# hupe1980/vecgo

Measured on AMD Instinct MI355X. Metric: QPS at recall@10≥0.95, 1M×768 HNSW+PQ; PQ-ADC HBM GB/s vs peak, higher is better.
Workload: dtype f32; 1 GPU; flat_exact_l2_1Mx768_top10 (BASELINE configs[1]): MFMA GEMM nomination + exact re-score + proof; operating_point=flat_exact, rows=1000000, dim=768, k=10, parallelism=1 GPU

## Files before the change

vecgo_amd/csrc/k_flat.hip:

```cpp
#include <algorithm>

#include "vg_device.hpp"
#include "vg_exact.hpp"
#include "vg_cand_replay.hpp"
#include "vg_flat_gemm.hpp"
#include "vg_internal.hpp"
#include "vg_nominate.hpp"
#include "vg_search.hpp"

namespace vg {

struct GemmOperands {
    const float *a, *b;
    int64_t n;
    int dim_words;
    const float *norms;
    bool bf16, dma;
};
struct NomCall {
    hipStream_t st;
    bool dot;
    GemmOperands ops;
    int64_t cnt;
    const uint8_t *mask;
// ... 4 lines not shown
    const NomCall &c;
    const float *queries;
    float *scores = nullptr;
    int tile_stride = 1;
    int64_t out_cols = 0;
    const float *thr = nullptr;
    int thr_stride = 0, thr_off = 0;
    int *counts = nullptr;
    uint64_t *cand = nullptr;
    int cap = 0;
    int cus = 256;
    int *counts_wide = nullptr;
    int skip_stride = 0;
    bool split = false;
    bool screen = false;
    const uint32_t *tile_active = nullptr;

    explicit GemmArgs(const NomCall &call) : c(call), queries(call.ops.a) {}
    static GemmArgs sample(const NomCall &c, float *sc, int stride, int64_t cols)
    {
        GemmArgs a(c);
        a.scores = sc, a.tile_stride = stride, a.out_cols = cols;
        return a;
    }
    static GemmArgs append(const NomCall &c, const float *thr, int sel_k, int *counts, uint64_t *cand, int cap)
    {
        GemmArgs a(c);
        a.thr = thr, a.thr_stride = sel_k, a.thr_off = sel_k - 1, a.counts = counts, a.cand = cand, a.cap = cap;
        return a;
    }
    GemmArgs &wide(int *lines, int compute_units) { return counts_wide = lines, cus = compute_units, *this; }
    GemmArgs &skipping(int stride) { return skip_stride = stride, *this; }
    GemmArgs &split_tile(const uint32_t *image) { return queries = reinterpret_cast<const float *>(image), split = true, *this; }
    GemmArgs &screen_tile() { return screen = true, *this; }
    GemmArgs &retry(const uint32_t *active) { return tile_active = active, *this; }
};
constexpr int kCountLine = 32;
static bool gemm_runs_split(bool fused, bool bf16, bool dma, int64_t nq, int dim, int cap, int thr_stride)
{
    return fused && !bf16 && dma && nq > kGemmBM && dim % kGemmBK == 0 && nq * static_cast<int64_t>(cap) < (int64_t(1) << 31) &&
           thr_stride < 65536 && !hook(kHookFlatNoSplit);
}
static float split_gemm_eps(bool dot, int dim)
{
    const float m = static_cast<float>(3 * dim + 16) * 5.9604645e-8f;
    return dot ? 1.5001f * 1.52587890625e-5f + 2.52f * m : 3.0002f * 1.52587890625e-5f + 4.03f * m;
}
static float screen_gemm_eps(bool dot, int dim)
{
    const float m = static_cast<float>(dim + 16) * 5.9604645e-8f;
    return dot ? 0.00390625f + 7.62939453125e-6f + 2.52f * m : 0.0078125f + 1.52587890625e-5f + 4.03f * m;
}
float bf16_filter_eps(bool dot) { return (dot ? 0.00390625f : 0.0078125f) * 1.02f; }
static bool gemm_skips_sample(bool dma, int64_t nq, bool bf16, bool split = false)
{
    if (bf16 || split || hook(kHookFlatRescoreSample)) return false;
    return !(dma && nq <= 3 * kG32BM && !hook(kHookFlatNoSmallTile));
}
__global__ void counts_narrow_kernel(const int *__restrict__ wide, int64_t nq, int *__restrict__ counts)
{
    const int64_t q = static_cast<int64_t>(blockIdx.x) * blockDim.x + threadIdx.x;
    if (q < nq) counts[q] = wide[q * kCountLine];
}

template <class Kern, class... Args>
static int32_t launch_lds(Kern kern, dim3 grid, dim3 threads, size_t lds, hipStream_t st, Args... args)
{
// ... 17 lines not shown
    const NomCall &c = a.c;
    const bool dma = c.ops.dma, bf16 = c.ops.bf16;
    const hipStream_t st = c.st;
    const int skip = MODE == 2 ? a.skip_stride : 0;
    VG_CHECK(skip == 0 || (skip > 1 && gemm_skips_sample(dma, c.cnt, bf16, a.split)), VG_ERR_INVALID_ARG, "launch_gemm: skip_stride on a kernel without it");
    const int64_t mt = (c.cnt + kGemmBM - 1) / kGemmBM, nt = (c.ops.n + kGemmBN - 1) / kGemmBN;
    const int64_t tiles = skip ? nt - gemm_skip_sampled_tiles(nt, skip) : (nt + a.tile_stride - 1) / a.tile_stride;
    const dim3 grid(static_cast<unsigned>(mt * ((tiles + 7) / 8) * 8)), threads(kGemmThreads);
    auto big_grid = [&](int64_t bnt ) {
        const int64_t bmt = (c.cnt + kBigBM - 1) / kBigBM;
        const int64_t slots = bmt * ((bnt + 7) / 8) * 8, per_cu = std::max(a.cus / 8, 1) * 8;
        return dim3(static_cast<unsigned>(std::min(slots, per_cu)));
    };
    auto launch_big = [&](auto kern, size_t lds, auto... extra) -> int32_t {
        if (a.counts_wide && !a.tile_active) VG_HIP(hipMemsetAsync(a.counts_wide, 0, sizeof(int) * static_cast<size_t>(c.cnt) * kCountLine, st));
        VG_TRY(launch_lds(kern, big_grid((c.ops.n + kBigBN - 1) / kBigBN), dim3(kBigThreads), lds, st, a.queries, c.cnt, c.ops.b, c.ops.n,
                          c.ops.dim_words, c.ops.norms, a.thr, a.thr_stride, a.thr_off, a.counts_wide ? a.counts_wide : a.counts, a.cand, a.cap, c.mask,
                          c.mask_stride, a.counts_wide ? kCountLine : 1, extra...));
        if (a.counts_wide)
            VG_LAUNCH(counts_narrow_kernel, dim3(static_cast<unsigned>((c.cnt + 255) / 256)), dim3(256), 0, st, a.counts_wide, c.cnt, a.counts);
        return VG_OK;
    };
    auto launch_tile = [&](auto kern, dim3 blocks, size_t lds, auto... last) -> int32_t {
        return launch_lds(kern, blocks, threads, lds, st, a.queries, c.cnt, c.ops.b, c.ops.n, c.ops.dim_words, c.ops.norms, a.scores, a.tile_stride, a.out_cols, a.thr,
                          a.thr_stride, a.thr_off, a.counts, a.cand, a.cap, c.mask, c.mask_stride, last...);
    };
    auto launch_128 = [&](auto kern, size_t lds, int last) { return launch_tile(kern, grid, lds, last); };
    auto launch_g32 = [&](auto kern, size_t lds) { return launch_tile(kern, dim3(static_cast<unsigned>(tiles)), lds); };
    constexpr int M = MODE == 0 ? 1 : MODE;
    const int rb = static_cast<int>((c.cnt + kG32BM - 1) / kG32BM);
    if constexpr (MODE == 1) {
        if (a.split) {
            VG_CHECK(!bf16 && gemm_runs_split(true, false, dma, c.cnt, c.ops.dim_words, 0, 0), VG_ERR_INVALID_ARG, "launch_gemm: sample tile on a call without it");
            return launch_lds(flat_gemm_sample_big_kernel<DOT, 3>, big_grid((tiles + 1) / 2), dim3(kBigThreads), big_lds_bytes<3>(), st, a.queries, c.cnt,
                              c.ops.b, c.ops.n, c.ops.dim_words, c.ops.norms, a.scores, a.tile_stride, a.out_cols, c.mask, c.mask_stride);
        }
    }
    if (MODE == 2 && a.split) {
        VG_CHECK(!bf16 && gemm_runs_split(true, false, dma, c.cnt, c.ops.dim_words, a.cap, a.thr_stride), VG_ERR_INVALID_ARG, "launch_gemm: split tile on a call without it");
        if (a.screen) return launch_big(flat_gemm_screen_big_kernel<DOT, 3>, big_lds_bytes<3>());
        VG_CHECK(!a.tile_active || (c.cnt <= 32 * kBigBM && a.counts_wide), VG_ERR_INVALID_ARG, "launch_gemm: tile_active is one word, with wide counters");
        note_flat_split_launch();
        return launch_big(flat_gemm_split_big_kernel<DOT, 3>, big_lds_bytes<3>(), a.tile_active);
    }
    if (skip && tiles == 0) return VG_OK;
    if (bf16) {
        if (c.cnt <= 4 * kG32BM && !hook(kHookFlatNoSmallTile)) return with_g32_tile<DOT, M, true>(rb, launch_g32);
        if (MODE == 2 && c.cnt > kGemmBM && c.cnt * static_cast<int64_t>(a.cap) < (int64_t(1) << 31) && a.thr_stride < 65536 &&
            !hook(kHookFlatNoBigTile)) {
            const bool two = hook(kHookFlatBigTile2);
            auto kern = two ? flat_gemm_bf16_big_kernel<DOT, 2> : hook(kHookFlatBigEarlyB) ? flat_gemm_bf16_big_kernel<DOT, 3, 512> : flat_gemm_bf16_big_kernel<DOT, 3>;
            return launch_big(kern, two ? big_lds_bytes<2>() : big_lds_bytes<3>());
        }
        return launch_128(flat_gemm_dma_kernel<DOT, M, 0, true>, kDmaLdsBytes, 0);
    }
    if (dma && MODE != 0 && c.cnt <= 3 * kG32BM && !hook(kHookFlatNoSmallTile)) return with_g32_tile<DOT, M, false>(rb, launch_g32);
    if (dma) return launch_128(flat_gemm_dma_kernel<DOT, MODE>, kDmaLdsBytes, skip);
    return launch_128(flat_gemm_kernel<DOT, MODE>, kGemmLdsBytes, skip);
}

template <int MODE>
static int32_t launch_gemm(const GemmArgs &a)
{
    return a.c.dot ? launch_gemm_t<true, MODE>(a) : launch_gemm_t<false, MODE>(a);
}

__global__ void f32_to_bf16_pad_kernel(const float *__restrict__ src, int64_t rows, int dim, int dim_pad, uint16_t *__restrict__ dst)
{
    const int64_t i = static_cast<int64_t>(blockIdx.x) * blockDim.x + threadIdx.x;
    if (i >= rows * dim_pad) return;
    const int64_t r = i / dim_pad;
    const int j = static_cast<int>(i - r * dim_pad);
    const uint32_t u = j < dim ? __float_as_uint(src[r * dim + j]) : 0u;
    uint16_t v;
    if ((u & 0x7F800000u) == 0x7F800000u && (u & 0x007FFFFFu) != 0)
        v = static_cast<uint16_t>((u >> 16) | 0x0040u);
    else
        v = static_cast<uint16_t>((u + 0x7FFFu + ((u >> 16) & 1u)) >> 16);
    dst[i] = v;
}

__global__ void flat_split_queries_kernel(const float *__restrict__ src, int64_t rows, int dim, uint32_t *__restrict__ dst)
{
    const int64_t i = static_cast<int64_t>(blockIdx.x) * blockDim.x + threadIdx.x;
    const int half = dim / 2;
    if (i >= rows * half) return;
    const int64_t r = i / half;
    const int p = static_cast<int>(i - r * half), s = p >> 4, w = p & 15;
    const float2 v = *reinterpret_cast<const float2 *>(src + r * dim + 32 * s + 2 * w);
    uint32_t hi, lo;
    split2_bf16(v.x, v.y, hi, lo);
    dst[r * dim + 32 * s + w] = hi;
    dst[r * dim + 32 * s + 16 + w] = lo;
}

__global__ __launch_bounds__(256) void flat_todo_kernel(const int *__restrict__ flags, const int *__restrict__ always,
                                                        int cnt, int *__restrict__ todo,
                                                        unsigned long long *__restrict__ stats, const int *__restrict__ counts)
{
    __shared__ int part[256];
    __shared__ unsigned long long appended[256];
    const int tid = threadIdx.x;
    const int per = (cnt + 255) / 256;
    const int lo = tid * per < cnt ? tid * per : cnt, hi = lo + per < cnt ? lo + per : cnt;
    if (!flags) {
        if (tid == 0) atomicAdd(&stats[0], static_cast<unsigned long long>(cnt));
        return;
    }
    const bool all = *always != 0;
    int mine = 0;
    unsigned long long app = 0;
    for (int i = lo; i < hi; i++) {
        mine += (all || flags[i] != 0);
        if (counts) app += static_cast<unsigned long long>(counts[i]);
    }
    part[tid] = mine;
    appended[tid] = app;
    __syncthreads();
    if (tid == 0) {
        int run = 0;
        app = 0;
        for (int t = 0; t < 256; t++) {
            const int c = part[t];
            part[t] = run;
            run += c;
            app += appended[t];
// ... 545 lines not shown
    {
        cols = cols_;
        slices = slices_ ? slices_ : select_slices(cols, 4096, 64);
        nom.sel_k = sel_k;
        nom.cap = cap;
        c.take(sc, sampled ? cnt * cols : 1);
        c.take(partial, cnt * slices * sel_k);
        c.take(sid, cnt * sel_k);
        c.take(nom.thr, cnt * sel_k);
        c.take(nom.counts, cnt);
        c.take(nom.cand, cnt * cap);
        c.take(nom.cand_id, cnt * kFlatKc);
        c.take(nom.cand_sc, cnt * kFlatKc);
    }
};
static int32_t launch_flat_select(const NomScratch &s, int64_t cnt, int sel_k, hipStream_t st)
{
    VG_LAUNCH(flat_select_kernel, dim3(s.slices, static_cast<unsigned>(cnt)), dim3(kSelThreads), 0, st, s.sc, s.cols, s.slices, sel_k, s.partial);
    return VG_OK;
}
static int32_t select_thresholds(const NomScratch &s, int64_t cnt, int sel_k, uint32_t *ids, float *thr, hipStream_t st)
{
    VG_TRY(launch_flat_select(s, cnt, sel_k, st));
    return launch_topk_merge(s.partial, cnt, s.slices, sel_k, false, ids, thr, st);
}
static int32_t sample_thresholds(const NomCall &c, const NomScratch &s, int stride, int sel_k, float *thr, bool sampled, const uint32_t *image = nullptr,
                                 int cus = 0)
{
    if (!sampled) {
        VG_LAUNCH(fill_f32_kernel, dim3(static_cast<unsigned>((c.cnt * sel_k + 255) / 256)), dim3(256), 0, c.st, thr, c.cnt * sel_k, INFINITY);
        return VG_OK;
    }
    GemmArgs a = GemmArgs::sample(c, s.sc, stride, s.cols);
    if (image) a.split_tile(image).wide(nullptr, cus);
    VG_TRY(launch_gemm<1>(a));
    return select_thresholds(s, c.cnt, sel_k, s.sid, thr, c.st);
}
static int32_t launch_flat_pick(const ProbeNominated &nom, int64_t cnt, const int *only, hipStream_t st)
{
    VG_LAUNCH(flat_pick_kernel, dim3(static_cast<unsigned>(cnt)), dim3(256), 0, st, nom.cand, nom.counts, nom.cap, kFlatKc, nom.cand_id, nom.cand_sc, only);
    return VG_OK;
}
static int32_t launch_flat_verify(bool dot, int k, const vg_index *idx, const float *queries, int64_t cnt, const ProbeNominated &nom,
                                  float eps_extra, uint32_t *ids, float *scores, int *fail, const int *only, hipStream_t st)
{
    return with_metric(dot, [&](auto dot_c) -> int32_t {
        constexpr bool DOT = decltype(dot_c)::value;
        const dim3 grid(static_cast<unsigned>(cnt)), threads(256);
        if (nom.thr && k > 64)
            VG_LAUNCH(flat_verify_sort_kernel<DOT>, grid, threads, sizeof(uint64_t) * static_cast<size_t>(nom.cap), st, idx->d_vectors, idx->dim, queries,
                      idx->d_norm_max, nom.cand, nom.counts, nom.cap, k, ids, scores, fail, nom.thr, nom.sel_k, nom.sel_k - 1, eps_extra);
        else if (nom.thr && k > kGemmMaxK)
            VG_LAUNCH(flat_verify_all_kernel<DOT>, grid, threads, 0, st, idx->d_vectors, idx->dim, queries, idx->d_norm_max, nom.cand, nom.counts,
                      nom.cap, k, ids, scores, fail, nom.thr, nom.sel_k, nom.sel_k - 1, eps_extra);
        else
            VG_LAUNCH(flat_verify_kernel<DOT>, grid, threads, 0, st, idx->d_vectors, idx->n, idx->dim, queries, idx->d_norm_max, nom.cand_id,
                      nom.cand_sc, kFlatKc, k, ids, scores, fail, nom.thr, nom.sel_k, nom.sel_k - 1, nom.counts, nom.cap, eps_extra, only);
        return VG_OK;
    });
}

struct FlatCall {
    vg_index *idx;
    int k;
    hipStream_t st;
    bool dot;
    const float *q;
    int64_t nq;
    const uint8_t *mask;
    int64_t mask_stride;
    uint32_t *oid;
    float *osc;
    int64_t n = idx->n;
    int dim = idx->dim;
    FlatCall range(int64_t q0, int64_t cnt) const
    {
        FlatCall r = *this;
        r.q += q0 * dim, r.nq = cnt, r.oid += q0 * k, r.osc += q0 * k;
        if (mask) r.mask += q0 * mask_stride;
        return r;
    }
    NomCall nom() const { return {st, dot, fp32_operands(idx, q, !hook(kHookFlatNoDma)), nq, mask, mask_stride}; }
};
constexpr int kFlatCap = 4096;
constexpr int kFlatSampleStride = 64;
static int exact_slices(int64_t n) { return static_cast<int>(std::min<int64_t>(256, std::max<int64_t>(1, n / 64))); }
struct FlatScratch : NomScratch {
    bool fused;
    bool use_sample;
    bool bf16;
    bool may_split;
    int ex_slices, pk;
    int64_t qc;
    int *flags, *todo;
    uint64_t *fpartial, *min_keys;
    uint32_t *fid;
    float *fsc;
    uint16_t *qbf;
    int *counts_wide;
    uint32_t *tile_active;
    FlatScratch(const FlatCall &c, bool unfused, char *base) : fused(!unfused), use_sample(fused && c.n > kFlatCap)
    {
        bf16 = c.idx->d_vectors_bf16 != nullptr && fused && !hook(kHookFlatNoDma);
        const int sel_k = !fused ? kFlatKc : c.k <= 64 ? 8 : std::min(64, std::max(8, (3 * c.k + 63) / 64));
        ex_slices = exact_slices(c.n);
        pk = std::min(c.k, 64);
        qc = fused ? 4096 : (int64_t(2) << 30) / (c.n * 4);
        if (qc > 4096) qc = 4096;
        if (qc >= kGemmBM) qc = (qc / kGemmBM) * kGemmBM;
        if (qc < 1) qc = 1;
        if (qc > c.nq) qc = c.nq;
        may_split = gemm_runs_split(fused, bf16, true, qc, c.dim, kFlatCap, sel_k);
        Carve cv{base};
        carve(cv, qc, fused ? sample_cols(c.n, kFlatSampleStride) : c.n, sel_k, fused ? kFlatCap : 0, !fused || use_sample);
        cv.take(flags, qc + 1);
        cv.take(todo, qc + 1);
        cv.take(fpartial, qc * ex_slices * pk);
        cv.take(fid, qc * pk);
        cv.take(fsc, qc * pk);
        cv.take(min_keys, qc);
        cv.take(qbf, bf16 ? qc * c.idx->vectors_bf16_dim : may_split ? 2 * qc * c.dim : 0);
        cv.take(counts_wide, bf16 || may_split ? qc * kCountLine : 0);
        cv.take(tile_active, may_split ? 1 : 0);
        bytes = cv.off;
    }
};

static int32_t flat_scan_small(const FlatCall &c)
{
    const int slices = static_cast<int>(std::min<int64_t>(4 * c.idx->ctx->compute_units, std::max<int64_t>(1, c.n / 64)));
    ArenaCall ar(c.idx->ctx, c.st);
    const int i_partial = ar.add(sizeof(uint64_t) * static_cast<size_t>(c.nq) * slices * c.k);
    VG_TRY(ar.commit());
    uint64_t *partial = ar.get<uint64_t>(i_partial);
    const size_t lds = sizeof(float) * static_cast<size_t>(kScanQB) * c.dim + 4 * 64 * sizeof(uint64_t) + 64;
    for (int64_t q0 = 0; q0 < c.nq; q0 += kScanQB) {
        const int cnt = static_cast<int>(std::min<int64_t>(kScanQB, c.nq - q0));
        ProfScope prof(c.idx->ctx, "flat_scan", c.st);
        auto kern = c.dot ? flat_scan_mq_kernel<true> : flat_scan_mq_kernel<false>;
        VG_LAUNCH(kern, dim3(slices), dim3(256), lds, c.st, c.idx->d_vectors, c.n, c.dim, c.q + q0 * c.dim, cnt, slices, c.k, partial + q0 * slices * c.k);
    }
    VG_TRY(launch_topk_merge(partial, c.nq, slices, c.k, c.dot, c.oid, c.osc, c.st));
    return launch_flat_todo(nullptr, nullptr, static_cast<int>(c.nq), nullptr, c.idx->d_flat_stats, c.st);
}

static int32_t launch_flat_exact(const FlatCall &c, const int *todo, int ex_slices, int kk, uint64_t *fpartial, const uint64_t *floor_keys)
{
    const unsigned slots = static_cast<unsigned>(std::min<int64_t>(c.nq, kExactSlots));
    auto kern = c.dot ? flat_exact_kernel<true> : flat_exact_kernel<false>;
    VG_LAUNCH(kern, dim3(ex_slices, slots), dim3(256), 0, c.st, c.idx->d_vectors, c.n, c.dim, c.q, todo, ex_slices, kk, fpartial, floor_keys, c.mask,
              c.mask_stride);
    return VG_OK;
}
static int32_t flat_exact_every_query(const FlatCall &call)
// ... 30 lines not shown
        VG_TRY(launch_flat_select(s, c.nq, kFlatKc, c.st));
    }
    VG_TRY(launch_topk_merge(s.partial, c.nq, s.slices, kFlatKc, false, s.nom.cand_id, s.nom.cand_sc, c.st));
    ProbeNominated nom = s.nom;
    nom.thr = nullptr;
    return launch_flat_verify(c.dot, c.k, c.idx, c.q, c.nq, nom, 0.0f, c.oid, c.osc, s.flags, nullptr, c.st);
}

static int32_t flat_screen_retry(const FlatCall &c, const NomCall &nc, const FlatScratch &s)
{
    const ProbeNominated &nom = s.nom;
    VG_LAUNCH(flat_retry_prepare_kernel, dim3(1), dim3(kBigBM), 0, c.st, s.flags, hook(kHookFlatScreenFail), static_cast<int>(c.nq), nom.thr,
              nom.sel_k, nom.sel_k - 1, nom.counts, s.counts_wide, s.tile_active, c.idx->d_flat_stats);
    {
        ProfScope prof(c.idx->ctx, "flat_retry", c.st);
        VG_TRY(launch_gemm<2>(GemmArgs::append(nc, nom.thr, nom.sel_k, nom.counts, nom.cand, nom.cap)
                                  .wide(s.counts_wide, c.idx->ctx->compute_units)
                                  .split_tile(reinterpret_cast<const uint32_t *>(s.qbf))
                                  .retry(s.tile_active)));
    }
    VG_TRY(launch_flat_pick(nom, c.nq, s.flags, c.st));
    return launch_flat_verify(c.dot, c.k, c.idx, c.q, c.nq, nom, split_gemm_eps(c.dot, c.dim), c.oid, c.osc, s.flags, s.flags, c.st);
}

static int32_t flat_fused_chunk(const FlatCall &c, const FlatScratch &s)
{
    const vg_index *idx = c.idx;
    const ProbeNominated &nom = s.nom;
    NomCall nc = c.nom();
    const bool split = gemm_runs_split(true, s.bf16, nc.ops.dma, c.nq, c.dim, nom.cap, nom.sel_k);
    const bool screen = gemm_runs_screen(split, c.k);
    const float eps_extra = screen ? screen_gemm_eps(c.dot, c.dim) : split ? split_gemm_eps(c.dot, c.dim) : s.bf16 ? bf16_filter_eps(c.dot) : 0.0f;
    if (s.bf16) VG_TRY(gemm_operands(c.q, c.nq, c.dim, c.n, idx->d_norms, idx->d_vectors_bf16, idx->vectors_bf16_dim, s.qbf, c.st, &nc.ops));
    const uint32_t *image = reinterpret_cast<const uint32_t *>(s.qbf);
    if (split)
        VG_LAUNCH(flat_split_queries_kernel, dim3(static_cast<unsigned>((c.nq * (c.dim / 2) + 255) / 256)), dim3(256), 0, c.st, c.q, c.nq, c.dim,
                  reinterpret_cast<uint32_t *>(s.qbf));
    VG_TRY(sample_thresholds(nc, s, kFlatSampleStride, nom.sel_k, nom.thr, s.use_sample, sample_runs_big(split, s.use_sample) ? image : nullptr,
                             idx->ctx->compute_units));
    if (s.bf16 || split) VG_LAUNCH(flat_thr_cap_kernel, dim3(nc.ucnt()), dim3(64), 0, c.st, nom.thr, nom.sel_k, c.q, c.dim, idx->d_norm_max);
    const bool once = s.use_sample && gemm_skips_sample(nc.ops.dma, c.nq, s.bf16, split);
    if (!once) VG_HIP(hipMemsetAsync(nom.counts, 0, sizeof(int) * static_cast<size_t>(c.nq), c.st));
    {
        ProfScope prof(idx->ctx, "flat_gemm", c.st);
        if (once)
            VG_LAUNCH(flat_sample_append_kernel, dim3(nc.ucnt()), dim3(kSampleAppendThreads), 0, c.st, s.sc, s.cols, kFlatSampleStride, nom.thr,
                      nom.sel_k, nom.sel_k - 1, nom.counts, nom.cand, nom.cap);
        GemmArgs a = GemmArgs::append(nc, nom.thr, nom.sel_k, nom.counts, nom.cand, nom.cap);
        a.wide(s.bf16 || split ? s.counts_wide : nullptr, idx->ctx->compute_units).skipping(once ? kFlatSampleStride : 0);
        if (split) a.split_tile(reinterpret_cast<const uint32_t *>(s.qbf));
        if (screen) a.screen_tile();
        VG_TRY(launch_gemm<2>(a));
    }
    if (c.k <= kGemmMaxK) VG_TRY(launch_flat_pick(nom, c.nq, nullptr, c.st));
    VG_TRY(launch_flat_verify(c.dot, c.k, idx, c.q, c.nq, nom, eps_extra, c.oid, c.osc, s.flags, nullptr, c.st));
    return screen ? flat_screen_retry(c, nc, s) : VG_OK;
}

static void flat_debug_counts(const FlatCall &c, int64_t q0, const FlatScratch &s)
{
    std::vector<int> hf(c.nq), hc(c.nq);
    (void)hipMemcpyAsync(hf.data(), s.flags, sizeof(int) * c.nq, hipMemcpyDeviceToHost, c.st);
    (void)hipMemcpyAsync(hc.data(), s.nom.counts, sizeof(int) * c.nq, hipMemcpyDeviceToHost, c.st);
    (void)hipStreamSynchronize(c.st);
    int64_t nf = 0, csum = 0, cmax = 0;
    for (int f : hf) nf += f != 0;
    for (int n : hc) { csum += n; cmax = std::max<int64_t>(cmax, n); }
    fprintf(stderr, "[vg_search_flat] chunk q0=%lld cnt=%lld: %lld queries failed the proof; "
            "appended candidates avg %.1f max %lld\n", (long long)q0, (long long)c.nq, (long long)nf,
            s.fused ? double(csum) / c.nq : 0.0, (long long)(s.fused ? cmax : 0));
}

static int32_t flat_fallback_pages(const FlatCall &c, const FlatScratch &s)
{
    const int *always = s.flags + s.qc;
    const dim3 grid(static_cast<unsigned>(c.nq));
    for (int off = 0; off < c.k; off += 64) {
        const int kk = std::min(64, c.k - off);
        VG_TRY(launch_flat_exact(c, s.todo, s.ex_slices, kk, s.fpartial, off ? s.min_keys : nullptr));
        VG_TRY(launch_topk_merge(s.fpartial, c.nq, s.ex_slices, kk, c.dot, s.fid, s.fsc, c.st, s.flags, always));
        if (c.k <= 64)
            VG_LAUNCH(flat_patch_kernel, grid, dim3(64), 0, c.st, s.flags, always, c.k, s.fid, s.fsc, c.oid, c.osc);
        else
            VG_LAUNCH(flat_page_patch_kernel, grid, dim3(64), 0, c.st, s.flags, always, c.k, off, kk, c.dot, s.fid, s.fsc, c.oid, c.osc, s.min_keys);
// ... 302 lines not shown
```

vecgo_amd/csrc/vg_flat_gemm.hpp:

```cpp
#pragma once

#include <hip/hip_runtime.h>

#include <cmath>
#include <cstdint>
#include <type_traits>

#include "vg_device.hpp"

namespace vg {

constexpr int kGemmBM = 128, kGemmBN = 128, kGemmBK = 32, kGemmLd = kGemmBK + 1;
constexpr int kGemmPasses = kGemmBM * kGemmBK / 4 / 256;
constexpr int kGemmThreads = 256;
constexpr int kGemmTile = kGemmBM * kGemmLd;
constexpr size_t kGemmLdsBytes = 4 * kGemmTile * sizeof(float);
using f32x16 = __attribute__((ext_vector_type(16))) float;

template <bool DOT, int MODE>
__device__ __forceinline__ void gemm_epilogue(const f32x16 (&acc)[2][2], float *lds_thr, float thr_reg,
                                              const float (&xn)[2], int tid, int lane, int wr, int wc, int64_t q0,
                                              int64_t nq, int64_t n0, int64_t n, int64_t tn,
                                              float *__restrict__ scores, int64_t out_cols,
                                              int *__restrict__ counts, uint64_t *__restrict__ cand, int cap,
// ... 438 lines not shown

struct GemmGroup {
    int64_t a_off, b_off;
    int32_t a_cnt, b_cnt;
};
template <bool DOT, int MODE, bool BF16 = false>
__global__ __launch_bounds__(kGemmThreads) void flat_gemm_dma_grouped_kernel(
    const GemmGroup *__restrict__ groups, const int64_t *__restrict__ first_block, int ngroups,
    const float *__restrict__ queries, const float *__restrict__ base, int dim, const float *__restrict__ norms,
    float *__restrict__ scores, int tile_stride, int64_t out_cols, const float *__restrict__ thr, int thr_stride, int thr_off,
    int *__restrict__ counts, uint64_t *__restrict__ cand, int cap, const uint8_t *__restrict__ mask , const int64_t *__restrict__ mask_off )
{
    const int64_t b = blockIdx.x;
    if (b >= first_block[ngroups]) return;
    int lo = 0, hi = ngroups - 1;
    while (lo < hi) {
        const int mid = (lo + hi + 1) >> 1;
        if (first_block[mid] <= b)
            lo = mid;
        else
            hi = mid - 1;
    }
    const GemmGroup g = groups[lo];
    if (g.a_cnt == 0 || g.b_cnt == 0) return;
    flat_gemm_dma_body<DOT, MODE, 0, BF16, true>(
        queries + g.a_off * dim, g.a_cnt, base + g.b_off * dim, g.b_cnt, dim, norms + g.b_off,
        scores ? scores + g.a_off * out_cols : nullptr, tile_stride, out_cols, thr ? thr + g.a_off * thr_stride : nullptr, thr_stride,
        thr_off, counts ? counts + g.a_off : nullptr, cand ? cand + g.a_off * cap : nullptr, cap, mask, 0, b - first_block[lo],
        static_cast<uint32_t>(g.b_off), mask ? mask_off + g.a_off : nullptr);
}

constexpr int kBigBM = 256, kBigBN = 256, kBigThreads = 512;
constexpr int kBigTile = kBigBM * kGemmBK;
template <int NB>
constexpr size_t big_lds_bytes() { return (2 + NB) * kBigTile * sizeof(float); }

__device__ __forceinline__ void big_split3(float x, uint32_t &p0, uint32_t &p1, uint32_t &p2)
{
    auto rne = [](float v) {
        const uint32_t u = __float_as_uint(v);
        return (u + 0x7FFFu + ((u >> 16) & 1u)) >> 16;
    };
    p0 = rne(x);
    const float r1 = x - __uint_as_float(p0 << 16);
    p1 = rne(r1);
    const float r2 = r1 - __uint_as_float(p1 << 16);
    p2 = rne(r2);
}
__device__ __forceinline__ int big_max3_i32(int a, int b, int c)
{
    int r;
    asm("v_max3_i32 %0, %1, %2, %3" : "=v"(r) : "v"(a), "v"(b), "v"(c));
    return r;
}

typedef __bf16 vg_bf16x2 __attribute__((ext_vector_type(2)));
typedef float vg_f32x2 __attribute__((ext_vector_type(2)));
__device__ __forceinline__ void split2_bf16(float a, float b, uint32_t &hi, uint32_t &lo)
{
    hi = __builtin_bit_cast(uint32_t, __builtin_convertvector(vg_f32x2{a, b}, vg_bf16x2));
    const float ra = a - __uint_as_float(hi << 16), rb = b - __uint_as_float(hi & 0xFFFF0000u);
    lo = __builtin_bit_cast(uint32_t, __builtin_convertvector(vg_f32x2{ra, rb}, vg_bf16x2));
}

enum { kBigImages = 0, kBigSplit = 1, kBigScreen = 2 };
template <bool DOT, int NB, int PROBE, int OPS, bool SAMPLE = false>
__device__ __forceinline__ void flat_gemm_big_body(
    const float *__restrict__ queries, int64_t nq, const float *__restrict__ base, int64_t n, int dim ,
    const float *__restrict__ norms, const float *__restrict__ thr, int thr_stride, int thr_off, int *__restrict__ counts,
    uint64_t *__restrict__ cand, int cap, const uint8_t *__restrict__ mask, int64_t mask_stride,
    int count_stride ,
    const uint32_t *__restrict__ tile_active = nullptr, float *__restrict__ scores = nullptr ,
    int tile_stride = 1, int64_t out_cols = 0)
{
    static_assert(NB == 2 || NB == 3, "two or three row-tile buffers");
    constexpr bool SPLIT = OPS != kBigImages;
    constexpr bool SCREEN = OPS == kBigScreen;
    extern __shared__ float gemm_lds[];
    const int mtiles = static_cast<int>((nq + kBigBM - 1) / kBigBM);
    const int ntiles = SAMPLE ? static_cast<int>((((n + kGemmBN - 1) / kGemmBN + tile_stride - 1) / tile_stride + 1) / 2)
                              : static_cast<int>((n + kBigBN - 1) / kBigBN);
    const int total = mtiles * ((ntiles + 7) / 8) * 8, G = static_cast<int>(gridDim.x), xcd = static_cast<int>(blockIdx.x & 7);
    const int dq = (G >> 3) / mtiles, dr = (G >> 3) % mtiles;
    struct Pos {
        int bt, quo, rem;
    };
    auto tm_of = [&](const Pos &p) { return p.rem; };
    auto tn_of = [&](const Pos &p) { return p.quo * 8 + xcd; };
    const uint32_t active = tile_active ? *tile_active : 0xFFFFFFFFu;
    auto hole = [&](const Pos &p) { return tn_of(p) >= ntiles || ((active >> (p.rem & 31)) & 1u) == 0; };
    auto step = [&](Pos &p) {
        do {
            p.bt += G;
            p.quo += dq;
            p.rem += dr;
            if (p.rem >= mtiles) {
                p.rem -= mtiles;
                p.quo++;
            }
        } while (p.bt < total && hole(p));
    };
    Pos pos0;
    pos0.bt = static_cast<int>(blockIdx.x);
    pos0.quo = (pos0.bt >> 3) / mtiles;
    pos0.rem = (pos0.bt >> 3) % mtiles;
    if (pos0.bt < total && hole(pos0)) step(pos0);
    if (pos0.bt >= total) return;
    int my_tiles = 0;
    for (Pos p = pos0; p.bt < total; step(p)) my_tiles++;

    const int tid = threadIdx.x;
    const int lane = tid & 63;
    const int wave = __builtin_amdgcn_readfirstlane(tid >> 6);
    const int wr = wave >> 2, wc = wave & 3;
    const int ksteps = dim / kGemmBK;
    const int S = my_tiles * ksteps;

    const int drow = wave * 8 + (lane >> 3);
    const int dgl = (lane & 7) ^ ((wave * 4 + (lane >> 4)) & 7);
    const uint32_t lds0 = static_cast<uint32_t>(reinterpret_cast<uintptr_t>(
        (__attribute__((address_space(3))) void *)gemm_lds));
    auto piece = [&](int buf, int p) {
        return static_cast<uint32_t>(__builtin_amdgcn_readfirstlane(
            static_cast<int>(lds0 + (buf * kBigTile + (p * 64 + wave * 8) * kGemmBK) * 4)));
    };
    Pos a_pos = pos0, b_pos = pos0;
    int a_k = 0, b_k = 0, ia = 0, ib = 0;
    const float *abase, *bbase, *bbase1 = nullptr;
    int a_last, b_last, b_last1 = 0;
    const uint32_t off0 = static_cast<uint32_t>((drow * dim + dgl * 4) * 4);
    auto set_a = [&](const Pos &ps) {
        const int64_t q0 = static_cast<int64_t>(tm_of(ps)) * kBigBM;
        abase = queries + q0 * dim;
        a_last = static_cast<int>(nq - q0 < kBigBM ? nq - q0 : kBigBM) - 1;
    };
    auto set_b = [&](const Pos &ps) {
        const int64_t n0 = static_cast<int64_t>(tn_of(ps)) * kBigBN;
        bbase = base + n0 * dim;
        b_last = static_cast<int>(n - n0 < kBigBN ? n - n0 : kBigBN) - 1;
    };
    auto half_row0 = [&](const Pos &ps, int hf) { return (static_cast<int64_t>(tn_of(ps)) * 2 + hf) * tile_stride * kGemmBN; };
    auto set_b_halves = [&](const Pos &ps) {
        const int64_t r0 = half_row0(ps, 0), r1 = half_row0(ps, 1);
        bbase = base + r0 * dim;
        b_last = static_cast<int>(n - r0 < kGemmBN ? n - r0 : kGemmBN) - 1;
        bbase1 = r1 < n ? base + r1 * dim : bbase;
        b_last1 = r1 < n ? static_cast<int>(n - r1 < kGemmBN ? n - r1 : kGemmBN) - 1 : b_last;
    };
    auto fill = [&](const float *src , int last, int buf) {
        if (last == kBigBM - 1) {
#pragma unroll
            for (int p = 0; p < 4; p++) glds16(src + static_cast<int64_t>(p) * 64 * dim, off0, piece(buf, p));
        } else {
#pragma unroll
            for (int p = 0; p < 4; p++) {
                const int row = p * 64 + drow < last ? p * 64 + drow : last;
                glds16(src, static_cast<uint32_t>((row * dim + dgl * 4) * 4), piece(buf, p));
            }
        }
    };
    auto fill_b = [&](int k0, int buf) {
        if constexpr (!SAMPLE) {
            fill(bbase + k0, b_last, buf);
        } else if (b_last == kGemmBN - 1 && b_last1 == kGemmBN - 1) {
#pragma unroll
            for (int p = 0; p < 4; p++) glds16((p < 2 ? bbase : bbase1) + k0 + static_cast<int64_t>(p & 1) * 64 * dim, off0, piece(buf, p));
        } else {
#pragma unroll
            for (int p = 0; p < 4; p++) {
                const int last = p < 2 ? b_last : b_last1;
                const int row = (p & 1) * 64 + drow < last ? (p & 1) * 64 + drow : last;
                glds16((p < 2 ? bbase : bbase1) + k0, static_cast<uint32_t>((row * dim + dgl * 4) * 4), piece(buf, p));
            }
        }
    };
    auto next_b = [&](const Pos &ps) {
        if constexpr (SAMPLE)
            set_b_halves(ps);
        else
            set_b(ps);
    };
    auto stage_a = [&]() {
        fill(abase + a_k * kGemmBK, a_last, ia);
        ia ^= 1;
        if (++a_k == ksteps) {
            a_k = 0;
            step(a_pos);
            if (a_pos.bt < total) set_a(a_pos);
        }
    };
    auto stage_b = [&]() {
        if (!(PROBE & 64)) fill_b(b_k * kGemmBK, 2 + ib);
        ib = ib + 1 == NB ? 0 : ib + 1;
        if (++b_k == ksteps) {
            b_k = 0;
            step(b_pos);
            if (b_pos.bt < total) next_b(b_pos);
        }
    };
    set_a(pos0);
    next_b(pos0);

    f32x16 acc[4][2];
    const int h = lane >> 5, f = (lane >> 1) & 7;
    int lpart[4];
#pragma unroll
    for (int j = 0; j < 4; j++) {
        const int gran = !SPLIT ? 2 * j + h : j < 2 ? 2 * j + h : 4 * (j - 2) + 2 * h;
        lpart[j] = (lane & 31) * kGemmBK + (gran ^ f) * 4;
    }
    const int a_wave = wr * 128 * kGemmBK, b_wave = wc * 64 * kGemmBK;

    constexpr float kThrClamp = 1e30f;
    Pos c_pos = pos0;
    float tq2[2], xq1;
    float xn[2] = {0.0f, 0.0f};
    auto tile_loads = [&](const Pos &ps) {
        if constexpr (SAMPLE) {
            const int64_t nn = half_row0(ps, wc >> 1) + (wc & 1) * 64 + lane;
            xq1 = norms[nn < n ? nn : n - 1];
            return;
        }
        const int64_t q0 = static_cast<int64_t>(tm_of(ps)) * kBigBM, n0 = static_cast<int64_t>(tn_of(ps)) * kBigBN;
#pragma unroll
        for (int i = 0; i < 2; i++) {
            const int64_t qq = q0 + wr * 128 + i * 64 + lane;
            tq2[i] = thr[(qq < nq ? qq : nq - 1) * thr_stride + thr_off];
        }
        const int64_t nn = n0 + wc * 64 + lane;
        xq1 = norms[nn < n ? nn : n - 1];
    };
    auto tile_init = [&]() {
        if constexpr (SAMPLE) {
#pragma unroll
            for (int i = 0; i < 4; i++)
#pragma unroll
                for (int j = 0; j < 2; j++)
#pragma unroll
                    for (int r = 0; r < 16; r++) acc[i][j][r] = 0.0f;
            return;
        }
        const uint32_t one = 0x3F80u;
        uint4 ta[4], xb[2];
        const int64_t iq0 = static_cast<int64_t>(tm_of(c_pos)) * kBigBM;
// ... 163 lines not shown
                        off += 4 * out_cols;
                        asm volatile("" : "+v"(off));
                        if (MASKED) __builtin_amdgcn_sched_barrier(0);
                    }
                }
            }
        };
        const bool whole = nq_in == kBigBM && (static_cast<int64_t>(tn_of(ps)) + 1) * kBigBN <= out_cols;
        if (mask == nullptr) {
            if (whole)
                put(std::false_type{}, std::false_type{});
            else
                put(std::true_type{}, std::false_type{});
        } else {
            if (whole)
                put(std::false_type{}, std::true_type{});
            else
                put(std::true_type{}, std::true_type{});
        }
        xn[0] = xnext[0], xn[1] = xnext[1];
    };

    float4 fa[2][4], fb[2][2];
    uint4 bc[2][2];
    auto read_part = [&](const float *As, const float *Bs, auto P) {
        constexpr int p = decltype(P)::value, set = p & 1;
        if constexpr (!SPLIT) {
            const float *pa = As + a_wave + lpart[p], *pb = Bs + b_wave + lpart[p];
#pragma unroll
            for (int i = 0; i < 4; i++) fa[set][i] = *reinterpret_cast<const float4 *>(pa + i * 32 * kGemmBK);
#pragma unroll
            for (int i = 0; i < 2; i++) fb[set][i] = *reinterpret_cast<const float4 *>(pb + i * 32 * kGemmBK);
        } else {
            const int oa = a_wave + lpart[p >> 1] + 2 * (p & 1) * 32 * kGemmBK;
#pragma unroll
            for (int b = 0; b < 2; b++) {
                fa[set][2 * b] = *reinterpret_cast<const float4 *>(As + oa + b * 32 * kGemmBK);
                if constexpr (!SCREEN) fa[set][2 * b + 1] = *reinterpret_cast<const float4 *>(As + ((oa + b * 32 * kGemmBK) ^ 16));
            }
            if constexpr ((p & 1) == 0) {
                const int ob = b_wave + lpart[2 + (p >> 1)];
#pragma unroll
                for (int b = 0; b < 2; b++) {
                    fb[b][0] = *reinterpret_cast<const float4 *>(Bs + ob + b * 32 * kGemmBK);
                    fb[b][1] = *reinterpret_cast<const float4 *>(Bs + ((ob + b * 32 * kGemmBK) ^ 4));
                }
            }
        }
    };
    auto mfma_part = [&](auto P) {
        constexpr int p = decltype(P)::value, set = p & 1;
        if constexpr (!SPLIT) {
#pragma unroll
            for (int i = 0; i < 4; i++)
#pragma unroll
                for (int j = 0; j < 2; j++)
                    acc[i][j] = __builtin_amdgcn_mfma_f32_32x32x16_bf16(__builtin_bit_cast(vg_bf16x8, fa[set][i]),
                                                                       __builtin_bit_cast(vg_bf16x8, fb[set][j]), acc[i][j], 0, 0, 0);
        } else {
            constexpr int i0 = 2 * (p & 1), even = (p & 1) == 0;
            auto raw = [&](int b, int w) { return w == 0 ? make_float2(fb[b][0].x, fb[b][0].y) : w == 1 ? make_float2(fb[b][0].z, fb[b][0].w) :
                                                  w == 2 ? make_float2(fb[b][1].x, fb[b][1].y) : make_float2(fb[b][1].z, fb[b][1].w); };
            auto put = [](uint4 &v, int w, uint32_t x) { (w == 0 ? v.x : w == 1 ? v.y : w == 2 ? v.z : v.w) = x; };
            auto get = [](const uint4 &v, int w) { return w == 0 ? v.x : w == 1 ? v.y : w == 2 ? v.z : v.w; };
            if constexpr (even) {
#pragma unroll
                for (int b = 0; b < 2; b++)
#pragma unroll
                    for (int w = 0; w < 4; w++)
                        put(bc[b][0], w, __builtin_bit_cast(uint32_t, __builtin_convertvector(vg_f32x2{raw(b, w).x, raw(b, w).y}, vg_bf16x2)));
                __builtin_amdgcn_sched_barrier(0);
// ... 8 lines not shown
                            __builtin_bit_cast(vg_bf16x8, fa[set][2 * b + (pr == 1 ? 1 : 0)]),
                            __builtin_bit_cast(vg_bf16x8, bc[j][pr == 2 ? 1 : 0]), acc[i0 + b][j], 0, 0, 0);
                        if constexpr (even && !SCREEN) {
                            if (pr < 2) {
                                const int u = pr * 4 + b * 2 + j, rb = u >> 2, w = u & 3;
                                const uint32_t hi = get(bc[rb][0], w);
                                const float ra = raw(rb, w).x - __uint_as_float(hi << 16), rc = raw(rb, w).y - __uint_as_float(hi & 0xFFFF0000u);
                                put(bc[rb][1], w, __builtin_bit_cast(uint32_t, __builtin_convertvector(vg_f32x2{ra, rc}, vg_bf16x2)));
                                __builtin_amdgcn_sched_barrier(0);
                            }
                        }
                    }
        }
    };
    using P0 = std::integral_constant<int, 0>;
    using P1 = std::integral_constant<int, 1>;
    using P2 = std::integral_constant<int, 2>;
    using P3 = std::integral_constant<int, 3>;

    tile_loads(pos0);
    stage_a();
    stage_b();
    if (NB == 3 && S > 1) stage_b();
    if constexpr (SAMPLE) pull_norms(xn);
    tile_init();
    if (NB == 3 && S > 1)
        asm volatile("s_waitcnt vmcnt(4)" ::: "memory");
    else
        asm volatile("s_waitcnt vmcnt(0)" ::: "memory");
    __builtin_amdgcn_s_barrier();
    asm volatile("" ::: "memory");
    int ra = 0, rb = 0;
    __builtin_amdgcn_s_waitcnt(0xC07F);
    read_part(gemm_lds, gemm_lds + 2 * kBigTile, P0{});
    int t = 0;
    for (int g = 0; g < S; g++) {
        const float *As = gemm_lds + ra * kBigTile, *Bs = gemm_lds + (2 + rb) * kBigTile;
        const bool last = t == ksteps - 1;
        Pos n_pos = c_pos;
        if (last) {
            step(n_pos);
            if (n_pos.bt >= total) n_pos = c_pos;
            tile_loads(n_pos);
        }
        if (!(PROBE & 16)) read_part(As, Bs, P1{});
        __builtin_amdgcn_sched_barrier(0);
        mfma_part(P0{});
        __builtin_amdgcn_sched_barrier(0);
        if (g + 1 < S && !(PROBE & 2)) stage_a();
        if (g + NB - 1 < S && !(PROBE & 2) && (PROBE & 512)) stage_b();
        if (!(PROBE & 16)) read_part(As, Bs, P2{});
        __builtin_amdgcn_sched_barrier(0);
        mfma_part(P1{});
        __builtin_amdgcn_sched_barrier(0);
        if (g + NB - 1 < S && !(PROBE & 2) && !(PROBE & 512)) stage_b();
        if (!(PROBE & 16)) read_part(As, Bs, P3{});
        __builtin_amdgcn_sched_barrier(0);
        mfma_part(P2{});
        __builtin_amdgcn_sched_barrier(0);
        ra ^= 1;
        rb = rb + 1 == NB ? 0 : rb + 1;
        __builtin_amdgcn_s_waitcnt(0xC07F);
        if (NB == 3 && g + 2 < S)
            asm volatile("s_waitcnt vmcnt(4)" ::: "memory");
        else
            asm volatile("s_waitcnt vmcnt(0)" ::: "memory");
        if (!(PROBE & 8)) __builtin_amdgcn_s_barrier();
        asm volatile("" ::: "memory");
        if (!(PROBE & 16)) read_part(gemm_lds + ra * kBigTile, gemm_lds + (2 + rb) * kBigTile, P0{});
        __builtin_amdgcn_sched_barrier(0);
        mfma_part(P3{});
        __builtin_amdgcn_sched_barrier(0);
        if (last) {
            if constexpr (SAMPLE) {
                tile_scores(c_pos);
            } else if (!(PROBE & 1)) {
                tile_append(c_pos);
            } else {
                float sum = 0.0f;
                for (int i = 0; i < 4; i++)
                    for (int j = 0; j < 2; j++)
                        for (int r = 0; r < 16; r++) sum += acc[i][j][r];
                if (sum == 123.456f) counts[0] = 1;
            }
            c_pos = n_pos;
            t = 0;
            if (PROBE & 1024) {
#pragma unroll
                for (int i = 0; i < 4; i++)
#pragma unroll
                    for (int j = 0; j < 2; j++)
#pragma unroll
                        for (int r = 0; r < 16; r++) acc[i][j][r] = 0.0f;
            } else {
                tile_init();
            }
        } else {
            t++;
        }
    }
    if constexpr (!SAMPLE) flush_parked();
    if ((PROBE & 32768) && lane == 0) atomicAdd(&counts[nq * count_stride], flushes);
// ... 254 lines not shown
```

Before: 477,100 queries/s.

## Pre-swizzle hi-only bf16 query image for screen GEMM to halve A staging

The query split kernel now also writes a separate hi-only bf16 image, padded to whole 256-row tiles and laid out per tile with an XOR swizzle. The screen GEMM kernel loads this compact image with direct 16-byte global-to-LDS copies and no row bounds handling, which halves its A-tile LDS footprint and global traffic. The change also marks several tile-scheduling scalars as wave-uniform with readfirstlane. The cost is an extra scratch buffer, a larger query split pass, and a second LDS addressing scheme that must stay consistent with the swizzle.

```diff
diff --git a/vecgo_amd/csrc/k_flat.hip b/vecgo_amd/csrc/k_flat.hip
--- a/vecgo_amd/csrc/k_flat.hip
+++ b/vecgo_amd/csrc/k_flat.hip
@@ -60,7 +60,8 @@
     GemmArgs &wide(int *lines, int compute_units) { return counts_wide = lines, cus = compute_units, *this; }
     GemmArgs &skipping(int stride) { return skip_stride = stride, *this; }
     GemmArgs &split_tile(const uint32_t *image) { return queries = reinterpret_cast<const float *>(image), split = true, *this; }
-    GemmArgs &screen_tile() { return screen = true, *this; }
+    GemmArgs &sample_tile(const uint32_t *hi_image) { return split_tile(hi_image); }
+    GemmArgs &screen_tile(const uint32_t *hi_image) { return split_tile(hi_image), screen = true, *this; }
     GemmArgs &retry(const uint32_t *active) { return tile_active = active, *this; }
 };
 constexpr int kCountLine = 32;
@@ -144,13 +145,13 @@
     if constexpr (MODE == 1) {
         if (a.split) {
             VG_CHECK(!bf16 && gemm_runs_split(true, false, dma, c.cnt, c.ops.dim_words, 0, 0), VG_ERR_INVALID_ARG, "launch_gemm: sample tile on a call without it");
-            return launch_lds(flat_gemm_sample_big_kernel<DOT, 3>, big_grid((tiles + 1) / 2), dim3(kBigThreads), big_lds_bytes<3>(), st, a.queries, c.cnt,
+            return launch_lds(flat_gemm_sample_big_kernel<DOT, 3>, big_grid((tiles + 1) / 2), dim3(kBigThreads), big_lds_bytes<3, true>(), st, a.queries, c.cnt,
                               c.ops.b, c.ops.n, c.ops.dim_words, c.ops.norms, a.scores, a.tile_stride, a.out_cols, c.mask, c.mask_stride);
         }
     }
     if (MODE == 2 && a.split) {
         VG_CHECK(!bf16 && gemm_runs_split(true, false, dma, c.cnt, c.ops.dim_words, a.cap, a.thr_stride), VG_ERR_INVALID_ARG, "launch_gemm: split tile on a call without it");
-        if (a.screen) return launch_big(flat_gemm_screen_big_kernel<DOT, 3>, big_lds_bytes<3>());
+        if (a.screen) return launch_big(flat_gemm_screen_big_kernel<DOT, 3>, big_lds_bytes<3, true>());
         VG_CHECK(!a.tile_active || (c.cnt <= 32 * kBigBM && a.counts_wide), VG_ERR_INVALID_ARG, "launch_gemm: tile_active is one word, with wide counters");
         note_flat_split_launch();
         return launch_big(flat_gemm_split_big_kernel<DOT, 3>, big_lds_bytes<3>(), a.tile_active);
@@ -192,18 +193,25 @@
     dst[i] = v;
 }
 
-__global__ void flat_split_queries_kernel(const float *__restrict__ src, int64_t rows, int dim, uint32_t *__restrict__ dst)
+static int64_t flat_hi_image_rows(int64_t rows) { return (rows + kBigBM - 1) / kBigBM * kBigBM; }
+__global__ void flat_split_queries_kernel(const float *__restrict__ src, int64_t rows, int dim, uint32_t *__restrict__ dst,
+                                          uint32_t *__restrict__ hi_dst)
 {
     const int64_t i = static_cast<int64_t>(blockIdx.x) * blockDim.x + threadIdx.x;
     const int half = dim / 2;
-    if (i >= rows * half) return;
     const int64_t r = i / half;
+    if (r >= (rows + kBigBM - 1) / kBigBM * kBigBM) return;
+    const int64_t rs = r < rows ? r : rows - 1;
     const int p = static_cast<int>(i - r * half), s = p >> 4, w = p & 15;
-    const float2 v = *reinterpret_cast<const float2 *>(src + r * dim + 32 * s + 2 * w);
+    const float2 v = *reinterpret_cast<const float2 *>(src + rs * dim + 32 * s + 2 * w);
     uint32_t hi, lo;
     split2_bf16(v.x, v.y, hi, lo);
-    dst[r * dim + 32 * s + w] = hi;
-    dst[r * dim + 32 * s + 16 + w] = lo;
+    if (r < rows) {
+        dst[r * dim + 32 * s + w] = hi;
+        dst[r * dim + 32 * s + 16 + w] = lo;
+    }
+    const int R = static_cast<int>(r & (kBigBM - 1));
+    hi_dst[((r / kBigBM) * (dim / 32) + s) * (kBigBM * 16) + R * 16 + (((w >> 2) ^ ((R >> 2) & 3)) << 2) + (w & 3)] = hi;
 }
 
 __global__ __launch_bounds__(256) void flat_todo_kernel(const int *__restrict__ flags, const int *__restrict__ always,
@@ -815,7 +823,7 @@
         return VG_OK;
     }
     GemmArgs a = GemmArgs::sample(c, s.sc, stride, s.cols);
-    if (image) a.split_tile(image).wide(nullptr, cus);
+    if (image) a.sample_tile(image).wide(nullptr, cus);
     VG_TRY(launch_gemm<1>(a));
     return select_thresholds(s, c.cnt, sel_k, s.sid, thr, c.st);
 }
@@ -880,6 +888,7 @@
     uint32_t *fid;
     float *fsc;
     uint16_t *qbf;
+    uint32_t *qhi;
     int *counts_wide;
     uint32_t *tile_active;
     FlatScratch(const FlatCall &c, bool unfused, char *base) : fused(!unfused), use_sample(fused && c.n > kFlatCap)
@@ -903,6 +912,7 @@
         cv.take(fsc, qc * pk);
         cv.take(min_keys, qc);
         cv.take(qbf, bf16 ? qc * c.idx->vectors_bf16_dim : may_split ? 2 * qc * c.dim : 0);
+        cv.take(qhi, may_split ? flat_hi_image_rows(qc) * (c.dim / 2) : 0);
         cv.take(counts_wide, bf16 || may_split ? qc * kCountLine : 0);
         cv.take(tile_active, may_split ? 1 : 0);
         bytes = cv.off;
@@ -999,11 +1009,10 @@
     const bool screen = gemm_runs_screen(split, c.k);
     const float eps_extra = screen ? screen_gemm_eps(c.dot, c.dim) : split ? split_gemm_eps(c.dot, c.dim) : s.bf16 ? bf16_filter_eps(c.dot) : 0.0f;
     if (s.bf16) VG_TRY(gemm_operands(c.q, c.nq, c.dim, c.n, idx->d_norms, idx->d_vectors_bf16, idx->vectors_bf16_dim, s.qbf, c.st, &nc.ops));
-    const uint32_t *image = reinterpret_cast<const uint32_t *>(s.qbf);
     if (split)
-        VG_LAUNCH(flat_split_queries_kernel, dim3(static_cast<unsigned>((c.nq * (c.dim / 2) + 255) / 256)), dim3(256), 0, c.st, c.q, c.nq, c.dim,
-                  reinterpret_cast<uint32_t *>(s.qbf));
-    VG_TRY(sample_thresholds(nc, s, kFlatSampleStride, nom.sel_k, nom.thr, s.use_sample, sample_runs_big(split, s.use_sample) ? image : nullptr,
+        VG_LAUNCH(flat_split_queries_kernel, dim3(static_cast<unsigned>((flat_hi_image_rows(c.nq) * (c.dim / 2) + 255) / 256)), dim3(256), 0, c.st, c.q,
+                  c.nq, c.dim, reinterpret_cast<uint32_t *>(s.qbf), s.qhi);
+    VG_TRY(sample_thresholds(nc, s, kFlatSampleStride, nom.sel_k, nom.thr, s.use_sample, sample_runs_big(split, s.use_sample) ? s.qhi : nullptr,
                              idx->ctx->compute_units));
     if (s.bf16 || split) VG_LAUNCH(flat_thr_cap_kernel, dim3(nc.ucnt()), dim3(64), 0, c.st, nom.thr, nom.sel_k, c.q, c.dim, idx->d_norm_max);
     const bool once = s.use_sample && gemm_skips_sample(nc.ops.dma, c.nq, s.bf16, split);
@@ -1015,8 +1024,10 @@
                       nom.sel_k, nom.sel_k - 1, nom.counts, nom.cand, nom.cap);
         GemmArgs a = GemmArgs::append(nc, nom.thr, nom.sel_k, nom.counts, nom.cand, nom.cap);
         a.wide(s.bf16 || split ? s.counts_wide : nullptr, idx->ctx->compute_units).skipping(once ? kFlatSampleStride : 0);
-        if (split) a.split_tile(reinterpret_cast<const uint32_t *>(s.qbf));
-        if (screen) a.screen_tile();
+        if (screen)
+            a.screen_tile(s.qhi);
+        else if (split)
+            a.split_tile(reinterpret_cast<const uint32_t *>(s.qbf));
         VG_TRY(launch_gemm<2>(a));
     }
     if (c.k <= kGemmMaxK) VG_TRY(launch_flat_pick(nom, c.nq, nullptr, c.st));
diff --git a/vecgo_amd/csrc/vg_flat_gemm.hpp b/vecgo_amd/csrc/vg_flat_gemm.hpp
--- a/vecgo_amd/csrc/vg_flat_gemm.hpp
+++ b/vecgo_amd/csrc/vg_flat_gemm.hpp
@@ -494,8 +494,9 @@
 
 constexpr int kBigBM = 256, kBigBN = 256, kBigThreads = 512;
 constexpr int kBigTile = kBigBM * kGemmBK;
-template <int NB>
-constexpr size_t big_lds_bytes() { return (2 + NB) * kBigTile * sizeof(float); }
+constexpr int kBigHiTile = kBigBM * kGemmBK / 2;
+template <int NB, bool HI = false>
+constexpr size_t big_lds_bytes() { return (2 * (HI ? kBigHiTile : kBigTile) + NB * kBigTile) * sizeof(float); }
 
 __device__ __forceinline__ void big_split3(float x, uint32_t &p0, uint32_t &p1, uint32_t &p2)
 {
@@ -540,10 +541,10 @@
     constexpr bool SCREEN = OPS == kBigScreen;
     extern __shared__ float gemm_lds[];
     const int mtiles = static_cast<int>((nq + kBigBM - 1) / kBigBM);
-    const int ntiles = SAMPLE ? static_cast<int>((((n + kGemmBN - 1) / kGemmBN + tile_stride - 1) / tile_stride + 1) / 2)
-                              : static_cast<int>((n + kBigBN - 1) / kBigBN);
+    const int ntiles = __builtin_amdgcn_readfirstlane(SAMPLE ? static_cast<int>((((n + kGemmBN - 1) / kGemmBN + tile_stride - 1) / tile_stride + 1) / 2)
+                                                             : static_cast<int>((n + kBigBN - 1) / kBigBN));
     const int total = mtiles * ((ntiles + 7) / 8) * 8, G = static_cast<int>(gridDim.x), xcd = static_cast<int>(blockIdx.x & 7);
-    const int dq = (G >> 3) / mtiles, dr = (G >> 3) % mtiles;
+    const int dq = __builtin_amdgcn_readfirstlane((G >> 3) / mtiles), dr = __builtin_amdgcn_readfirstlane((G >> 3) % mtiles);
     struct Pos {
         int bt, quo, rem;
     };
@@ -564,8 +565,8 @@
     };
     Pos pos0;
     pos0.bt = static_cast<int>(blockIdx.x);
-    pos0.quo = (pos0.bt >> 3) / mtiles;
-    pos0.rem = (pos0.bt >> 3) % mtiles;
+    pos0.quo = __builtin_amdgcn_readfirstlane((pos0.bt >> 3) / mtiles);
+    pos0.rem = __builtin_amdgcn_readfirstlane((pos0.bt >> 3) % mtiles);
     if (pos0.bt < total && hole(pos0)) step(pos0);
     if (pos0.bt >= total) return;
     int my_tiles = 0;
@@ -582,9 +583,12 @@
     const int dgl = (lane & 7) ^ ((wave * 4 + (lane >> 4)) & 7);
     const uint32_t lds0 = static_cast<uint32_t>(reinterpret_cast<uintptr_t>(
         (__attribute__((address_space(3))) void *)gemm_lds));
+    constexpr int kATile = SCREEN ? kBigHiTile : kBigTile, kARow = SCREEN ? kGemmBK / 2 : kGemmBK;
+    auto a_buf = [&](int i) { return i * kATile; };
+    auto b_buf = [&](int i) { return 2 * kATile + i * kBigTile; };
     auto piece = [&](int buf, int p) {
         return static_cast<uint32_t>(__builtin_amdgcn_readfirstlane(
-            static_cast<int>(lds0 + (buf * kBigTile + (p * 64 + wave * 8) * kGemmBK) * 4)));
+            static_cast<int>(lds0 + (buf + (p * 64 + wave * 8) * kGemmBK) * 4)));
     };
     Pos a_pos = pos0, b_pos = pos0;
     int a_k = 0, b_k = 0, ia = 0, ib = 0;
@@ -593,7 +597,7 @@
     const uint32_t off0 = static_cast<uint32_t>((drow * dim + dgl * 4) * 4);
     auto set_a = [&](const Pos &ps) {
         const int64_t q0 = static_cast<int64_t>(tm_of(ps)) * kBigBM;
-        abase = queries + q0 * dim;
+        abase = queries + (SCREEN ? q0 * (dim / 2) : q0 * dim);
         a_last = static_cast<int>(nq - q0 < kBigBM ? nq - q0 : kBigBM) - 1;
     };
     auto set_b = [&](const Pos &ps) {
@@ -643,7 +647,15 @@
             set_b(ps);
     };
     auto stage_a = [&]() {
-        fill(abase + a_k * kGemmBK, a_last, ia);
+        if constexpr (SCREEN) {
+            int t16 = tid;
+            asm volatile("" : "+v"(t16));
+            t16 *= 16;
+#pragma unroll
+            for (int p = 0; p < 2; p++) glds16(abase + a_k * kBigHiTile + p * 64 * kGemmBK, static_cast<uint32_t>(t16), piece(a_buf(ia), p));
+        } else {
+            fill(abase + a_k * kGemmBK, a_last, a_buf(ia));
+        }
         ia ^= 1;
         if (++a_k == ksteps) {
             a_k = 0;
@@ -652,7 +664,7 @@
         }
     };
     auto stage_b = [&]() {
-        if (!(PROBE & 64)) fill_b(b_k * kGemmBK, 2 + ib);
+        if (!(PROBE & 64)) fill_b(b_k * kGemmBK, b_buf(ib));
         ib = ib + 1 == NB ? 0 : ib + 1;
         if (++b_k == ksteps) {
             b_k = 0;
@@ -670,8 +682,9 @@
     for (int j = 0; j < 4; j++) {
         const int gran = !SPLIT ? 2 * j + h : j < 2 ? 2 * j + h : 4 * (j - 2) + 2 * h;
         lpart[j] = (lane & 31) * kGemmBK + (gran ^ f) * 4;
-    }
-    const int a_wave = wr * 128 * kGemmBK, b_wave = wc * 64 * kGemmBK;
+        if (SCREEN && j < 2) lpart[j] = (lane & 31) * kARow + (gran ^ ((lane >> 2) & 3)) * 4;
+    }
+    const int a_wave = wr * 128 * kARow, b_wave = wc * 64 * kGemmBK;
 
     constexpr float kThrClamp = 1e30f;
     Pos c_pos = pos0;
@@ -901,11 +914,11 @@
 #pragma unroll
             for (int i = 0; i < 2; i++) fb[set][i] = *reinterpret_cast<const float4 *>(pb + i * 32 * kGemmBK);
         } else {
-            const int oa = a_wave + lpart[p >> 1] + 2 * (p & 1) * 32 * kGemmBK;
+            const int oa = a_wave + (SCREEN ? lpart[0] ^ (8 * (p >> 1)) : lpart[p >> 1]) + 2 * (p & 1) * 32 * kARow;
 #pragma unroll
             for (int b = 0; b < 2; b++) {
-                fa[set][2 * b] = *reinterpret_cast<const float4 *>(As + oa + b * 32 * kGemmBK);
-                if constexpr (!SCREEN) fa[set][2 * b + 1] = *reinterpret_cast<const float4 *>(As + ((oa + b * 32 * kGemmBK) ^ 16));
+                fa[set][2 * b] = *reinterpret_cast<const float4 *>(As + oa + b * 32 * kARow);
+                if constexpr (!SCREEN) fa[set][2 * b + 1] = *reinterpret_cast<const float4 *>(As + ((oa + b * 32 * kARow) ^ 16));
             }
             if constexpr ((p & 1) == 0) {
                 const int ob = b_wave + lpart[2 + (p >> 1)];
@@ -980,10 +993,10 @@
     asm volatile("" ::: "memory");
     int ra = 0, rb = 0;
     __builtin_amdgcn_s_waitcnt(0xC07F);
-    read_part(gemm_lds, gemm_lds + 2 * kBigTile, P0{});
+    read_part(gemm_lds + a_buf(0), gemm_lds + b_buf(0), P0{});
     int t = 0;
     for (int g = 0; g < S; g++) {
-        const float *As = gemm_lds + ra * kBigTile, *Bs = gemm_lds + (2 + rb) * kBigTile;
+        const float *As = gemm_lds + a_buf(ra), *Bs = gemm_lds + b_buf(rb);
         const bool last = t == ksteps - 1;
         Pos n_pos = c_pos;
         if (last) {
@@ -1015,7 +1028,7 @@
             asm volatile("s_waitcnt vmcnt(0)" ::: "memory");
         if (!(PROBE & 8)) __builtin_amdgcn_s_barrier();
         asm volatile("" ::: "memory");
-        if (!(PROBE & 16)) read_part(gemm_lds + ra * kBigTile, gemm_lds + (2 + rb) * kBigTile, P0{});
+        if (!(PROBE & 16)) read_part(gemm_lds + a_buf(ra), gemm_lds + b_buf(rb), P0{});
         __builtin_amdgcn_sched_barrier(0);
         mfma_part(P3{});
         __builtin_amdgcn_sched_barrier(0);
```

New measurement: 522,200 queries/s (median of 6 runs). +9.4%, better.
